# Haochen-Wang409/U2PL

Measured on AMD Instinct MI355X. Metric: train images/sec at 769x769 (R101-DeepLabv3+), higher is better.
Workload: dtype f32

## Files before the change

### u2pl_amd/csrc/common.h

```cpp
#pragma once
#include <hip/hip_runtime.h>
#include <stdint.h>

#define U2PL_API extern "C" __attribute__((visibility("default")))

#define U2PL_LAUNCH_CHECK()                      \
    do {                                         \
        hipError_t e__ = hipGetLastError();      \
        if (e__ != hipSuccess) return (int)e__;  \
    } while (0)

#define U2PL_EINVAL 1001

#include <atomic>
extern std::atomic<unsigned long long> u2pl_kernel_launch_count;
#define U2PL_LAUNCH(...)                        \
    do {                                        \
        u2pl_kernel_launch_count.fetch_add(1, std::memory_order_relaxed);             \
        hipLaunchKernelGGL(__VA_ARGS__);        \
    } while (0)

#ifdef U2PL_HBM_MAXW
#define U2PL_HBM_KERNEL __attribute__((amdgpu_waves_per_eu(1, U2PL_HBM_MAXW)))
#else
#define U2PL_HBM_KERNEL
#endif

static inline int cdiv(long a, long b) { return (int)((a + b - 1) / b); }
static inline int grid_for(long n, int block, int max_blocks = 256 * 16) {
    long g = (n + block - 1) / block;
    if (g > max_blocks) g = max_blocks;
    if (g < 1) g = 1;
    return (int)g;
}

__device__ __forceinline__ float wave_sum(float v) {
#pragma unroll
    for (int o = 32; o > 0; o >>= 1) v += __shfl_xor(v, o, 64);
    return v;
}
template <int CTRL>
__device__ __forceinline__ float dpp_add(float v) {
    return v + __builtin_bit_cast(float, __builtin_amdgcn_update_dpp(0, __builtin_bit_cast(int, v), CTRL, 0xf, 0xf, false));
}
__device__ __forceinline__ float wave_allsum_dpp(float v) {
    v = dpp_add<0x128>(v);
    v = dpp_add<0x124>(v);
    v = dpp_add<0x122>(v);
    v = dpp_add<0x121>(v);
    const int b = __builtin_bit_cast(int, v);
    const float r0 = __builtin_bit_cast(float, __builtin_amdgcn_readlane(b, 0)), r1 = __builtin_bit_cast(float, __builtin_amdgcn_readlane(b, 16));
    const float r2 = __builtin_bit_cast(float, __builtin_amdgcn_readlane(b, 32)), r3 = __builtin_bit_cast(float, __builtin_amdgcn_readlane(b, 48));
    return (r0 + r1) + (r2 + r3);
}
__device__ __forceinline__ float wave_sum_sgpr(float v) {
    v = dpp_add<0x128>(v);
    v = dpp_add<0x124>(v);
    v = dpp_add<0x122>(v);
    v = dpp_add<0x121>(v);
    v += __builtin_bit_cast(float, __builtin_amdgcn_update_dpp(0, __builtin_bit_cast(int, v), 0x142, 0xa, 0xf, false));
    v += __builtin_bit_cast(float, __builtin_amdgcn_update_dpp(0, __builtin_bit_cast(int, v), 0x143, 0xc, 0xf, false));
    return __builtin_bit_cast(float, __builtin_amdgcn_readlane(__builtin_bit_cast(int, v), 63));
}
__device__ __forceinline__ float lane_put(float old, float val, int lane) {
    return (int)(threadIdx.x & 63) == lane ? val : old;
}
__device__ __forceinline__ float lane_get(float v, int lane) {
    return __builtin_bit_cast(float, __builtin_amdgcn_readlane(__builtin_bit_cast(int, v), lane));
}
__device__ __forceinline__ double wave_sum_d(double v) {
#pragma unroll
    for (int o = 32; o > 0; o >>= 1) v += __shfl_xor(v, o, 64);
    return v;
}
__device__ __forceinline__ unsigned wave_sum_u(unsigned v) {
#pragma unroll
    for (int o = 32; o > 0; o >>= 1) v += __shfl_xor(v, o, 64);
    return v;
}
__device__ __forceinline__ float wave_max(float v) {
#pragma unroll
    for (int o = 32; o > 0; o >>= 1) v = fmaxf(v, __shfl_xor(v, o, 64));
    return v;
}

#define U2PL_AMAX_SHARDS 64
#define U2PL_AMAX_STRIDE 32
#define U2PL_AMAX_WORDS (U2PL_AMAX_SHARDS * U2PL_AMAX_STRIDE)
__device__ __forceinline__ unsigned amax_bits(unsigned m, float v) {
    const unsigned b = __float_as_uint(v) & 0x7fffffffu;
    return b > m ? b : m;
}
__device__ __forceinline__ unsigned amax_bits4(unsigned m, float4 v) {
    return amax_bits(amax_bits(amax_bits(amax_bits(m, v.x), v.y), v.z), v.w);
}
__device__ __forceinline__ unsigned wave_max_u(unsigned m) {
#pragma unroll
    for (int o = 32; o > 0; o >>= 1) {
        const unsigned t = (unsigned)__shfl_xor((int)m, o, 64);
        m = t > m ? t : m;
    }
    return m;
}
__device__ __forceinline__ void amax_wave_publish(unsigned m, unsigned* __restrict__ obj) {
    m = wave_max_u(m);
    if ((threadIdx.x & 63) == 0 && m != 0u) {
        const unsigned wave = blockIdx.x * (blockDim.x >> 6) + (threadIdx.x >> 6);
        atomicMax(obj + (wave & (U2PL_AMAX_SHARDS - 1)) * U2PL_AMAX_STRIDE, m);
    }
}
__device__ __forceinline__ unsigned amax_read(const unsigned* __restrict__ obj) {
    const unsigned v = *(const __attribute__((address_space(1))) unsigned*)(obj + (threadIdx.x & 63) * U2PL_AMAX_STRIDE);
    return (unsigned)__builtin_amdgcn_readfirstlane((int)wave_max_u(v));
}

__device__ __forceinline__ void block_count_flush(unsigned cnt, unsigned* __restrict__ dst) {
    __shared__ unsigned s_cnt;
    if (threadIdx.x == 0) s_cnt = 0;
    __syncthreads();
    cnt = wave_sum_u(cnt);
    if ((threadIdx.x & 63) == 0 && cnt) atomicAdd(&s_cnt, cnt);
    __syncthreads();
    if (threadIdx.x == 0 && s_cnt) atomicAdd(dst, s_cnt);
}

__device__ __forceinline__ unsigned f32_key(float f) {
    unsigned u = __float_as_uint(f);
    return (u & 0x80000000u) ? ~u : (u | 0x80000000u);
}
__device__ __forceinline__ float key_f32(unsigned k) {
    unsigned u = (k & 0x80000000u) ? (k & 0x7fffffffu) : ~k;
    return __uint_as_float(u);
}

struct AcCoord {
    int i0, i1;
    float l0, l1;
};
__device__ __forceinline__ AcCoord ac_coord(int dst, float scale, int in_size) {
    AcCoord c;
    float src = __fmul_rn((float)dst, scale);
    c.i0 = (int)src;
    if (c.i0 > in_size - 1) c.i0 = in_size - 1;
    c.i1 = c.i0 + (c.i0 < in_size - 1 ? 1 : 0);
    c.l1 = __fsub_rn(src, (float)c.i0);
    c.l0 = __fsub_rn(1.0f, c.l1);
    return c;
}
static inline float ac_scale_host(long in, long out) {
    return out > 1 ? (float)(in - 1) / (float)(out - 1) : 0.0f;
}
__device__ __forceinline__ int nearest_src(int dst, float scale, int in_size) {
    int s = (int)floorf(__fmul_rn((float)dst, scale));
    return s < in_size - 1 ? s : in_size - 1;
}

typedef unsigned int u32x4 __attribute__((ext_vector_type(4)));
#define OOB_OFF ((int)0x80000000u)
__device__ __forceinline__ __amdgpu_buffer_rsrc_t make_rsrc(const void* p, unsigned bytes) {
    return __builtin_amdgcn_make_buffer_rsrc((void*)p, (short)0, (int)bytes, 0x00020000);
}
__device__ __forceinline__ float4 buf_load4s(__amdgpu_buffer_rsrc_t r, int lane_off, int uniform_off) {
    u32x4 v = __builtin_amdgcn_raw_buffer_load_b128(r, lane_off, uniform_off, 0);
    return make_float4(__uint_as_float(v.x), __uint_as_float(v.y), __uint_as_float(v.z), __uint_as_float(v.w));
}
__device__ __forceinline__ float4 buf_load4(__amdgpu_buffer_rsrc_t r, int byte_off) {
    u32x4 v = __builtin_amdgcn_raw_buffer_load_b128(r, byte_off, 0, 0);
    return make_float4(__uint_as_float(v.x), __uint_as_float(v.y), __uint_as_float(v.z), __uint_as_float(v.w));
}

#define U2PL_GLOBAL __attribute__((address_space(1)))
template <class T>
__device__ __forceinline__ T ldg(const T* p) { return *(const U2PL_GLOBAL T*)p; }

struct BnEpi {
    const float *mean, *invstd, *gamma, *beta, *res;
    long ldr;
    int relu;
    unsigned* y_amax;
};
```

### u2pl_amd/csrc/wino.hip

```cpp
#include "common.h"
#include "u2pl_hip.h"
#include "wino_t.h"

struct WinoGeom {
    int N, H, W, C, dil, Ty, Tx;
    long tiles;
};

__device__ __forceinline__ void tile_coords(const WinoGeom& g, long t, int& n, int& py, int& px, int& ty, int& tx) {
    tx = (int)(t % g.Tx); t /= g.Tx;
    ty = (int)(t % g.Ty); t /= g.Ty;
    px = (int)(t % g.dil); t /= g.dil;
    py = (int)(t % g.dil);
    n = (int)(t / g.dil);
}

template <int MT>
__global__ __launch_bounds__(256) U2PL_HBM_KERNEL void k_wino_input(const float* __restrict__ x, long ldx, unsigned xbytes, WinoGeom g,
                                                    float* __restrict__ V, unsigned* __restrict__ v_amax) {
    constexpr int A = WinoT<MT>::A;
    const int C4 = g.C >> 2;
    long idx = blockIdx.x * (long)blockDim.x + threadIdx.x;
    if (idx >= g.tiles * C4) {
        if (!v_amax) return;
        idx = g.tiles * C4 - 1;
    }
    const int c4 = (int)(idx % C4);
    const long t = idx / C4;
    int n, py, px, ty, tx;
    tile_coords(g, t, n, py, px, ty, tx);
    const __amdgpu_buffer_rsrc_t rx = make_rsrc(x, xbytes);
    const int ldxb = (int)ldx * 4;
    const int iy0 = py + g.dil * (ty * MT - 1), ix0 = px + g.dil * (tx * MT - 1);
    float4 d[A][A];
#pragma unroll
    for (int i = 0; i < A; ++i) {
        const int iy = iy0 + i * g.dil;
        const bool oky = iy >= 0 && iy < g.H;
#pragma unroll
        for (int j = 0; j < A; ++j) {
            const int ix = ix0 + j * g.dil;
            const bool ok = oky && ix >= 0 && ix < g.W;
            const int off = ((n * g.H + iy) * g.W + ix) * ldxb + c4 * 16;
            d[i][j] = buf_load4(rx, ok ? off : OOB_OFF);
        }
    }
#pragma unroll
    for (int j = 0; j < A; ++j) {
        float4 col[A], r[A];
#pragma unroll
        for (int i = 0; i < A; ++i) col[i] = d[i][j];
        WinoT<MT>::bt(col, r);
#pragma unroll
        for (int i = 0; i < A; ++i) d[i][j] = r[i];
    }
    const long comp_stride = g.tiles * (long)g.C;
    float* out = V + t * g.C + c4 * 4;
    unsigned am = 0u;
#pragma unroll
    for (int i = 0; i < A; ++i) {
        float4 r[A];
        WinoT<MT>::bt(d[i], r);
#pragma unroll
        for (int j = 0; j < A; ++j) {
            *(float4*)(out + (long)(i * A + j) * comp_stride) = r[j];
            am = amax_bits4(am, r[j]);
        }
    }
    if (v_amax) amax_wave_publish(am, v_amax);
}

template <int MT>
__device__ __forceinline__ void wino_weight_one(const float* __restrict__ w, int O, int C, int transposed, float* __restrict__ U, long idx) {
    constexpr int A = WinoT<MT>::A;
    const int c = transposed ? (int)(idx / O) : (int)(idx % C), o = transposed ? (int)(idx % O) : (int)(idx / C);
    float gk[3][3];
#pragma unroll
    for (int r = 0; r < 3; ++r)
#pragma unroll
        for (int s = 0; s < 3; ++s) {
            const int rr = transposed ? 2 - r : r, ss = transposed ? 2 - s : s;
            gk[r][s] = w[(((long)o * 3 + rr) * 3 + ss) * C + c];
        }
    float t[A][3];
#pragma unroll
    for (int s = 0; s < 3; ++s) {
        float col[3] = {gk[0][s], gk[1][s], gk[2][s]}, r[A];
        WinoT<MT>::gg(col, r);
#pragma unroll
        for (int i = 0; i < A; ++i) t[i][s] = r[i];
    }
    const long comp_stride = (long)O * C;
    const long base = transposed ? (long)c * O + o : (long)o * C + c;
#pragma unroll
    for (int i = 0; i < A; ++i) {
        float r[A];
        WinoT<MT>::gg(t[i], r);
#pragma unroll
        for (int j = 0; j < A; ++j) U[(long)(i * A + j) * comp_stride + base] = r[j];
    }
}
template <int MT>
__global__ void k_wino_weight(const float* __restrict__ w, int O, int C, int transposed, float* __restrict__ U) {
    const long idx = blockIdx.x * (long)blockDim.x + threadIdx.x;
    if (idx >= (long)O * C) return;
    wino_weight_one<MT>(w, O, C, transposed, U, idx);
}
struct WinoWeightJob { const float* w; float* U; long begin; int O, C, transposed, mt; };
__global__ void k_wino_weight_multi(const WinoWeightJob* __restrict__ jobs, int njobs, long total) {
    for (long i = blockIdx.x * (long)blockDim.x + threadIdx.x; i < total; i += (long)gridDim.x * blockDim.x) {
        int lo = 0, hi = njobs - 1;
        while (lo < hi) {
            const int mid = (lo + hi + 1) >> 1;
            if (jobs[mid].begin <= i) lo = mid; else hi = mid - 1;
        }
        const WinoWeightJob j = jobs[lo];
        if (j.mt == 4) wino_weight_one<4>(j.w, j.O, j.C, j.transposed, j.U, i - j.begin);
        else wino_weight_one<2>(j.w, j.O, j.C, j.transposed, j.U, i - j.begin);
    }
}

template <int MT>
__global__ __launch_bounds__(256) U2PL_HBM_KERNEL void k_wino_output(const float* __restrict__ Mb, WinoGeom g, int O,
                                                     const float* __restrict__ bias, float* __restrict__ y, long ldy,
                                                     float* __restrict__ stats, const float* __restrict__ pivot,
                                                     BnEpi epi) {
    constexpr int A = WinoT<MT>::A;
    __shared__ __attribute__((aligned(16))) float red[2][256][4];
    const int O4 = O >> 2;
    const int tpb = 256 / O4 > 0 ? 256 / O4 : 1;
    long t;
    int o4;
    bool live;
    if (stats) {
        o4 = threadIdx.x % O4;
        const int tl = threadIdx.x / O4;
        t = (long)blockIdx.x * tpb + tl;
        live = tl < tpb && t < g.tiles;
    } else {
        const long idx = blockIdx.x * (long)blockDim.x + threadIdx.x;
        o4 = (int)(idx % O4);
        t = idx / O4;
        live = t < g.tiles;
    }
    float4 s1 = make_float4(0.f, 0.f, 0.f, 0.f), s2 = s1;
    unsigned am = 0u;
    if (live) {
        int n, py, px, ty, tx;
        tile_coords(g, t, n, py, px, ty, tx);
        const long comp_stride = g.tiles * (long)O;
        const float* in = Mb + t * O + o4 * 4;
        float4 m[A][A];
#pragma unroll
        for (int i = 0; i < A; ++i)
#pragma unroll
            for (int j = 0; j < A; ++j) m[i][j] = *(const float4*)(in + (long)(i * A + j) * comp_stride);
        float4 tmp[MT][A];
#pragma unroll
        for (int j = 0; j < A; ++j) {
            float4 col[A], r[MT];
#pragma unroll
            for (int i = 0; i < A; ++i) col[i] = m[i][j];
            WinoT<MT>::at(col, r);
#pragma unroll
            for (int i = 0; i < MT; ++i) tmp[i][j] = r[i];
        }
        const float* bp = bias + o4 * 4;
        const float* pp = pivot + o4 * 4;
        const float4 bv = bias ? make_float4(bp[0], bp[1], bp[2], bp[3]) : make_float4(0.f, 0.f, 0.f, 0.f);
        const float4 pv = (stats && pivot) ? make_float4(pp[0], pp[1], pp[2], pp[3]) : make_float4(0.f, 0.f, 0.f, 0.f);
        const bool bn_on = epi.mean != nullptr;
        float4 mu4 = bv, is4 = bv, ga4 = bv, be4 = bv;
        if (bn_on) {
            mu4 = *(const float4*)(epi.mean + o4 * 4); is4 = *(const float4*)(epi.invstd + o4 * 4);
            ga4 = *(const float4*)(epi.gamma + o4 * 4); be4 = *(const float4*)(epi.beta + o4 * 4);
        }
#pragma unroll
        for (int i = 0; i < MT; ++i) {
            float4 r[MT];
            WinoT<MT>::at(tmp[i], r);
            const int oy = py + g.dil * (ty * MT + i);
#pragma unroll
            for (int j = 0; j < MT; ++j) {
                const int ox = px + g.dil * (tx * MT + j);
                if (oy < g.H && ox < g.W) {
                    float4 v = f4add(r[j], bv);
                    const long pix = (long)(n * g.H + oy) * g.W + ox;
                    if (bn_on) {
                        v.x = (v.x - mu4.x) * is4.x * ga4.x + be4.x; v.y = (v.y - mu4.y) * is4.y * ga4.y + be4.y;
                        v.z = (v.z - mu4.z) * is4.z * ga4.z + be4.z; v.w = (v.w - mu4.w) * is4.w * ga4.w + be4.w;
                        if (epi.res) v = f4add(v, *(const float4*)(epi.res + pix * epi.ldr + o4 * 4));
                        if (epi.relu) { v.x = fmaxf(v.x, 0.f); v.y = fmaxf(v.y, 0.f); v.z = fmaxf(v.z, 0.f); v.w = fmaxf(v.w, 0.f); }
                    }
                    *(float4*)(y + pix * ldy + o4 * 4) = v;
                    am = amax_bits4(am, v);
                    const float4 dv = f4sub(v, pv);
                    s1 = f4add(s1, dv);
                    s2 = f4add(s2, make_float4(dv.x * dv.x, dv.y * dv.y, dv.z * dv.z, dv.w * dv.w));
                }
            }
        }
    }
    if (epi.y_amax) amax_wave_publish(am, epi.y_amax);
    if (!stats) return;
    *(float4*)red[0][threadIdx.x] = s1;
    *(float4*)red[1][threadIdx.x] = s2;
    __syncthreads();
    for (int c = threadIdx.x; c < O; c += 256) {
        float a1 = 0.f, a2 = 0.f;
        for (int tl = 0; tl < tpb; ++tl) {
            a1 += red[0][tl * O4 + (c >> 2)][c & 3];
            a2 += red[1][tl * O4 + (c >> 2)][c & 3];
        }
        stats[(long)blockIdx.x * 2 * O + c] = a1;
        stats[(long)blockIdx.x * 2 * O + O + c] = a2;
    }
}

template <int MT>
__global__ __launch_bounds__(256) U2PL_HBM_KERNEL void k_wino_gy(const float* __restrict__ gy, long ldg, unsigned gbytes, WinoGeom g,
                                                 float* __restrict__ Mg, unsigned* __restrict__ mg_amax) {
    constexpr int A = WinoT<MT>::A;
    const int C4 = g.C >> 2;
    long idx = blockIdx.x * (long)blockDim.x + threadIdx.x;
    if (idx >= g.tiles * C4) {
        if (!mg_amax) return;
        idx = g.tiles * C4 - 1;
    }
    const int c4 = (int)(idx % C4);
    const long t = idx / C4;
    int n, py, px, ty, tx;
    tile_coords(g, t, n, py, px, ty, tx);
    const __amdgpu_buffer_rsrc_t rg = make_rsrc(gy, gbytes);
    const int ldb = (int)ldg * 4;
    float4 v[MT][MT];
#pragma unroll
    for (int i = 0; i < MT; ++i) {
        const int oy = py + g.dil * (ty * MT + i);
#pragma unroll
        for (int j = 0; j < MT; ++j) {
            const int ox = px + g.dil * (tx * MT + j);
            const bool ok = oy < g.H && ox < g.W;
            const int off = ((n * g.H + oy) * g.W + ox) * ldb + c4 * 16;
            v[i][j] = buf_load4(rg, ok ? off : OOB_OFF);
        }
    }
    float4 tmp[A][MT];
#pragma unroll
    for (int j = 0; j < MT; ++j) {
        float4 col[MT], r[A];
#pragma unroll
        for (int i = 0; i < MT; ++i) col[i] = v[i][j];
        WinoT<MT>::av(col, r);
#pragma unroll
        for (int i = 0; i < A; ++i) tmp[i][j] = r[i];
    }
    const long comp_stride = g.tiles * (long)g.C;
    float* out = Mg + t * g.C + c4 * 4;
    unsigned am = 0u;
#pragma unroll
    for (int i = 0; i < A; ++i) {
        float4 r[A];
        WinoT<MT>::av(tmp[i], r);
#pragma unroll
        for (int j = 0; j < A; ++j) {
            *(float4*)(out + (long)(i * A + j) * comp_stride) = r[j];
            am = amax_bits4(am, r[j]);
        }
    }
    if (mg_amax) amax_wave_publish(am, mg_amax);
}

template <int MT>
__global__ __launch_bounds__(256) void k_wino_wgrad_finish(const float* __restrict__ part, int nsplit, int O, int C,
                                                           int accumulate, float* __restrict__ dw) {
    constexpr int A = WinoT<MT>::A;
    const int C4 = C >> 2;
    const long idx = blockIdx.x * (long)blockDim.x + threadIdx.x;
    if (idx >= (long)O * C4) return;
    const int c4 = (int)(idx % C4), o = (int)(idx / C4);
    const long slab = (long)O * A * A * C;
    const float* p = part + (long)o * A * A * C + c4 * 4;
    float4 u[A][A];
#pragma unroll
    for (int i = 0; i < A; ++i)
#pragma unroll
        for (int j = 0; j < A; ++j) u[i][j] = make_float4(0.f, 0.f, 0.f, 0.f);
    for (int z = 0; z < nsplit; ++z) {
        float4 v[A][A];
#pragma unroll
        for (int i = 0; i < A; ++i)
#pragma unroll
            for (int j = 0; j < A; ++j) v[i][j] = *(const float4*)(p + (long)z * slab + (long)(i * A + j) * C);
#pragma unroll
        for (int i = 0; i < A; ++i)
#pragma unroll
            for (int j = 0; j < A; ++j) u[i][j] = f4add(u[i][j], v[i][j]);
    }
    float4 t[3][A];
#pragma unroll
    for (int j = 0; j < A; ++j) {
        float cx[A], cy[A], cz[A], cw[A], rx[3], ry[3], rz[3], rw[3];
#pragma unroll
        for (int i = 0; i < A; ++i) { cx[i] = u[i][j].x; cy[i] = u[i][j].y; cz[i] = u[i][j].z; cw[i] = u[i][j].w; }
        WinoT<MT>::gt(cx, rx); WinoT<MT>::gt(cy, ry); WinoT<MT>::gt(cz, rz); WinoT<MT>::gt(cw, rw);
#pragma unroll
        for (int i = 0; i < 3; ++i) t[i][j] = make_float4(rx[i], ry[i], rz[i], rw[i]);
    }
    const bool vec_ok = (reinterpret_cast<uintptr_t>(dw) & 15) == 0;
#pragma unroll
    for (int r3 = 0; r3 < 3; ++r3) {
        float cx[A], cy[A], cz[A], cw[A], rx[3], ry[3], rz[3], rw[3];
#pragma unroll
        for (int j = 0; j < A; ++j) { cx[j] = t[r3][j].x; cy[j] = t[r3][j].y; cz[j] = t[r3][j].z; cw[j] = t[r3][j].w; }
        WinoT<MT>::gt(cx, rx); WinoT<MT>::gt(cy, ry); WinoT<MT>::gt(cz, rz); WinoT<MT>::gt(cw, rw);
#pragma unroll
        for (int s3 = 0; s3 < 3; ++s3) {
            float* d = dw + (((long)o * 3 + r3) * 3 + s3) * C + c4 * 4;
            float4 val = make_float4(rx[s3], ry[s3], rz[s3], rw[s3]);
            if (vec_ok) {
                if (accumulate) val = f4add(*(const float4*)d, val);
                *(float4*)d = val;
            } else {
                d[0] = accumulate ? d[0] + val.x : val.x; d[1] = accumulate ? d[1] + val.y : val.y;
                d[2] = accumulate ? d[2] + val.z : val.z; d[3] = accumulate ? d[3] + val.w : val.w;
            }
        }
    }
}

static int wino_geom(int N, int H, int W, int C, int dil, int mt, WinoGeom& g) {
    if (mt != 2 && mt != 4) return U2PL_EINVAL;
    if (dil < 1 || C % 4) return U2PL_EINVAL;
    g.N = N; g.H = H; g.W = W; g.C = C; g.dil = dil;
    g.Ty = cdiv(cdiv(H, dil), mt);
    g.Tx = cdiv(cdiv(W, dil), mt);
    g.tiles = (long)N * dil * dil * g.Ty * g.Tx;
    return 0;
}

U2PL_API size_t u2pl_wino_tiles(int N, int H, int W, int dil, int mt) {
    WinoGeom g;
    if (wino_geom(N, H, W, 4, dil, mt, g)) return 0;
    return (size_t)g.tiles;
}
U2PL_API int u2pl_wino_stat_blocks(long tiles, int O) {
    const int tpb = 256 / (O / 4) > 0 ? 256 / (O / 4) : 1;
    return (int)((tiles + tpb - 1) / tpb);
}

static int run_wino_input(const float* x, long ldx, int N, int H, int W, int C, int dil, int mt, float* V, float* v_amax,
                          hipStream_t stream) {
    WinoGeom g;
    if (wino_geom(N, H, W, C, dil, mt, g)) return U2PL_EINVAL;
    const long xb = (((long)N * H * W - 1) * ldx + C) * 4;
    if (xb >= (1L << 31)) return U2PL_EINVAL;
    const long total = g.tiles * (C / 4);
    const dim3 grid((unsigned)cdiv(total, 256)), block(256);
    if (mt == 4) U2PL_LAUNCH(k_wino_input<4>, grid, block, 0, stream, x, ldx, (unsigned)xb, g, V, (unsigned*)v_amax);
    else U2PL_LAUNCH(k_wino_input<2>, grid, block, 0, stream, x, ldx, (unsigned)xb, g, V, (unsigned*)v_amax);
    U2PL_LAUNCH_CHECK();
    return 0;
}
U2PL_API int u2pl_wino_input_f32(const float* x, long ldx, int N, int H, int W, int C, int dil, int mt, float* V,
                                 hipStream_t stream) {
    return run_wino_input(x, ldx, N, H, W, C, dil, mt, V, nullptr, stream);
}
U2PL_API int u2pl_wino_input_amax_f32(const float* x, long ldx, int N, int H, int W, int C, int dil, int mt, float* V, float* v_amax,
                                      hipStream_t stream) {
    return run_wino_input(x, ldx, N, H, W, C, dil, mt, V, v_amax, stream);
}

U2PL_API int u2pl_wino_weight_multi_f32(const void* jobs, int njobs, long total, hipStream_t stream) {
    if (njobs <= 0 || total <= 0) return njobs == 0 ? 0 : U2PL_EINVAL;
    U2PL_LAUNCH(k_wino_weight_multi, dim3(grid_for(total, 256, 4096)), dim3(256), 0, stream, (const WinoWeightJob*)jobs, njobs, total);
    U2PL_LAUNCH_CHECK();
    return 0;
}
U2PL_API int u2pl_wino_weight_f32(const float* w, int O, int C, int transposed, int mt, float* U, hipStream_t stream) {
    if (mt != 2 && mt != 4) return U2PL_EINVAL;
    const dim3 grid((unsigned)cdiv((long)O * C, 256)), block(256);
    if (mt == 4) U2PL_LAUNCH(k_wino_weight<4>, grid, block, 0, stream, w, O, C, transposed, U);
    else U2PL_LAUNCH(k_wino_weight<2>, grid, block, 0, stream, w, O, C, transposed, U);
    U2PL_LAUNCH_CHECK();
    return 0;
}

static int run_wino_output(const float* Mb, int N, int H, int W, int O, int dil, int mt, const float* bias, float* y,
                           long ldy, float* stats_partial, const float* pivot, const BnEpi& epi, hipStream_t stream) {
    WinoGeom g;
    if (wino_geom(N, H, W, O, dil, mt, g)) return U2PL_EINVAL;
    if (stats_partial && (O / 4 > 256 || (O & 3))) return U2PL_EINVAL;
    const long total = g.tiles * (O / 4);
    const unsigned nblk = stats_partial ? (unsigned)u2pl_wino_stat_blocks(g.tiles, O) : (unsigned)cdiv(total, 256);
    if (mt == 4) U2PL_LAUNCH(k_wino_output<4>, dim3(nblk), dim3(256), 0, stream, Mb, g, O, bias, y, ldy, stats_partial, pivot, epi);
    else U2PL_LAUNCH(k_wino_output<2>, dim3(nblk), dim3(256), 0, stream, Mb, g, O, bias, y, ldy, stats_partial, pivot, epi);
    U2PL_LAUNCH_CHECK();
    return 0;
}
U2PL_API int u2pl_wino_output_f32(const float* Mb, int N, int H, int W, int O, int dil, int mt, const float* bias,
                                  float* y, long ldy, float* stats_partial, const float* pivot, hipStream_t stream) {
    const BnEpi off = {nullptr, nullptr, nullptr, nullptr, nullptr, 0, 0, nullptr};
    return run_wino_output(Mb, N, H, W, O, dil, mt, bias, y, ldy, stats_partial, pivot, off, stream);
}
U2PL_API int u2pl_wino_output_bnact_f32(const float* Mb, int N, int H, int W, int O, int dil, int mt, const float* bias,
                                        float* y, long ldy, const float* mean, const float* invstd, const float* gamma,
                                        const float* beta, const float* res, long ldr, int relu, hipStream_t stream) {
    if (!mean || !invstd || !gamma || !beta || (O & 3) || (ldy & 3) || (res && (ldr & 3))) return U2PL_EINVAL;
    const BnEpi epi = {mean, invstd, gamma, beta, res, ldr, relu, nullptr};
    return run_wino_output(Mb, N, H, W, O, dil, mt, bias, y, ldy, nullptr, nullptr, epi, stream);
}
U2PL_API int u2pl_wino_output_bnact_amax_f32(const float* Mb, int N, int H, int W, int O, int dil, int mt, const float* bias,
                                             float* y, long ldy, const float* mean, const float* invstd, const float* gamma,
                                             const float* beta, const float* res, long ldr, int relu, float* y_amax,
                                             hipStream_t stream) {
    if (!mean || !invstd || !gamma || !beta || (O & 3) || (ldy & 3) || (res && (ldr & 3))) return U2PL_EINVAL;
    const BnEpi epi = {mean, invstd, gamma, beta, res, ldr, relu, (unsigned*)y_amax};
    return run_wino_output(Mb, N, H, W, O, dil, mt, bias, y, ldy, nullptr, nullptr, epi, stream);
}

static int run_wino_gy(const float* gy, long ldg, int N, int H, int W, int O, int dil, int mt, float* Mg, float* mg_amax,
                       hipStream_t stream) {
    WinoGeom g;
    if (wino_geom(N, H, W, O, dil, mt, g)) return U2PL_EINVAL;
    const long gb = (((long)N * H * W - 1) * ldg + O) * 4;
    if (gb >= (1L << 31)) return U2PL_EINVAL;
    const long total = g.tiles * (O / 4);
    const dim3 grid((unsigned)cdiv(total, 256)), block(256);
    if (mt == 4) U2PL_LAUNCH(k_wino_gy<4>, grid, block, 0, stream, gy, ldg, (unsigned)gb, g, Mg, (unsigned*)mg_amax);
    else U2PL_LAUNCH(k_wino_gy<2>, grid, block, 0, stream, gy, ldg, (unsigned)gb, g, Mg, (unsigned*)mg_amax);
    U2PL_LAUNCH_CHECK();
    return 0;
}
U2PL_API int u2pl_wino_gy_f32(const float* gy, long ldg, int N, int H, int W, int O, int dil, int mt, float* Mg,
                              hipStream_t stream) {
    return run_wino_gy(gy, ldg, N, H, W, O, dil, mt, Mg, nullptr, stream);
}
U2PL_API int u2pl_wino_gy_amax_f32(const float* gy, long ldg, int N, int H, int W, int O, int dil, int mt, float* Mg, float* mg_amax,
                                   hipStream_t stream) {
    return run_wino_gy(gy, ldg, N, H, W, O, dil, mt, Mg, mg_amax, stream);
}

U2PL_API int u2pl_wino_wgrad_finish_f32(const float* part, int nsplit, int O, int C, int mt, int accumulate, float* dw,
                                        hipStream_t stream) {
    if (mt != 2 && mt != 4) return U2PL_EINVAL;
    if (C % 4) return U2PL_EINVAL;
    const dim3 grid((unsigned)cdiv((long)O * (C / 4), 256)), block(256);
    if (mt == 4) U2PL_LAUNCH(k_wino_wgrad_finish<4>, grid, block, 0, stream, part, nsplit, O, C, accumulate, dw);
    else U2PL_LAUNCH(k_wino_wgrad_finish<2>, grid, block, 0, stream, part, nsplit, O, C, accumulate, dw);
    U2PL_LAUNCH_CHECK();
    return 0;
}
```

Before: 38.29.

## Specialize Winograd input/output kernels with compile-time variants, 32-bit indexing, buffer ops

Templates the Winograd input and output transform kernels on wave-uniform tile ownership, amax and epilogue form, so unused branches (stats, BN, residual, amax) compile away. Index math moves from 64-bit to 32-bit, and the tile index is made scalar via readfirstlane when every wave owns a single tile, which enables scalar-offset buffer loads. Output stores use buffer stores with OOB masking instead of branches, and launch bounds set occupancy targets. In exchange there are more kernel instantiations and new size guards that reject tensors whose offsets exceed 32 bits.

Result: no change. 38.05 (-0.6%).

```diff
diff --git a/u2pl_amd/csrc/common.h b/u2pl_amd/csrc/common.h
--- a/u2pl_amd/csrc/common.h
+++ b/u2pl_amd/csrc/common.h
@@ -169,6 +169,12 @@
     return make_float4(__uint_as_float(v.x), __uint_as_float(v.y), __uint_as_float(v.z), __uint_as_float(v.w));
 }
 
+__device__ __forceinline__ void buf_store4(__amdgpu_buffer_rsrc_t r, int byte_off, float4 v) {
+    u32x4 w;
+    w.x = __float_as_uint(v.x); w.y = __float_as_uint(v.y); w.z = __float_as_uint(v.z); w.w = __float_as_uint(v.w);
+    __builtin_amdgcn_raw_buffer_store_b128(w, r, byte_off, 0, 0);
+}
+
 #define U2PL_GLOBAL __attribute__((address_space(1)))
 template <class T>
 __device__ __forceinline__ T ldg(const T* p) { return *(const U2PL_GLOBAL T*)p; }
diff --git a/u2pl_amd/csrc/wino.hip b/u2pl_amd/csrc/wino.hip
--- a/u2pl_amd/csrc/wino.hip
+++ b/u2pl_amd/csrc/wino.hip
@@ -1,12 +1,29 @@
 #include "common.h"
 #include "u2pl_hip.h"
 #include "wino_t.h"
+#include <type_traits>
 
 struct WinoGeom {
     int N, H, W, C, dil, Ty, Tx;
     long tiles;
 };
 
+#ifdef U2PL_HBM_MAXW
+#define U2PL_WINO_KERNEL(W) __launch_bounds__(256) U2PL_HBM_KERNEL
+#else
+#define U2PL_WINO_KERNEL(W) __launch_bounds__(256, W)
+#endif
+
+__device__ __forceinline__ void tile_coords(const WinoGeom& g, unsigned t, int& n, int& py, int& px, int& ty, int& tx) {
+    const unsigned r = t / (unsigned)g.Tx, q = r / (unsigned)g.Ty;
+    tx = (int)(t - r * (unsigned)g.Tx);
+    ty = (int)(r - q * (unsigned)g.Ty);
+    if (g.dil == 1) { px = 0; py = 0; n = (int)q; return; }
+    const unsigned u = q / (unsigned)g.dil;
+    px = (int)(q - u * (unsigned)g.dil);
+    n = (int)(u / (unsigned)g.dil);
+    py = (int)(u - (unsigned)n * (unsigned)g.dil);
+}
 __device__ __forceinline__ void tile_coords(const WinoGeom& g, long t, int& n, int& py, int& px, int& ty, int& tx) {
     tx = (int)(t % g.Tx); t /= g.Tx;
     ty = (int)(t % g.Ty); t /= g.Ty;
@@ -14,19 +31,36 @@
     py = (int)(t % g.dil);
     n = (int)(t / g.dil);
 }
-
-template <int MT>
-__global__ __launch_bounds__(256) U2PL_HBM_KERNEL void k_wino_input(const float* __restrict__ x, long ldx, unsigned xbytes, WinoGeom g,
+template <bool UNI>
+__device__ __forceinline__ unsigned wave_tile(unsigned t) {
+    return UNI ? (unsigned)__builtin_amdgcn_readfirstlane((int)t) : t;
+}
+typedef float f32x4g __attribute__((ext_vector_type(4)));
+__device__ __forceinline__ float4 plane_load4(const float* base, unsigned long plane, int k, unsigned off) {
+    const f32x4g v = *(const U2PL_GLOBAL f32x4g*)((const U2PL_GLOBAL char*)base + (unsigned long)k * plane + off);
+    return make_float4(v.x, v.y, v.z, v.w);
+}
+__device__ __forceinline__ float4 f4sel(bool c, float4 a, float4 b) {
+    return make_float4(c ? a.x : b.x, c ? a.y : b.y, c ? a.z : b.z, c ? a.w : b.w);
+}
+__device__ __forceinline__ float4 ldg4f(const float* p) { return plane_load4(p, 0, 0, 0u); }
+__device__ __forceinline__ void plane_store4(float* base, unsigned long plane, int k, unsigned off, float4 v) {
+    f32x4g w; w.x = v.x; w.y = v.y; w.z = v.z; w.w = v.w;
+    *(U2PL_GLOBAL f32x4g*)((U2PL_GLOBAL char*)base + (unsigned long)k * plane + off) = w;
+}
+
+template <int MT, bool UNI, bool AMAX>
+__global__ U2PL_WINO_KERNEL(MT == 4 ? 2 : 6) void k_wino_input(const float* __restrict__ x, long ldx, unsigned xbytes, WinoGeom g,
                                                     float* __restrict__ V, unsigned* __restrict__ v_amax) {
     constexpr int A = WinoT<MT>::A;
-    const int C4 = g.C >> 2;
-    long idx = blockIdx.x * (long)blockDim.x + threadIdx.x;
-    if (idx >= g.tiles * C4) {
-        if (!v_amax) return;
-        idx = g.tiles * C4 - 1;
-    }
-    const int c4 = (int)(idx % C4);
-    const long t = idx / C4;
+    const unsigned C4 = (unsigned)g.C >> 2, total = (unsigned)g.tiles * C4;
+    unsigned idx = blockIdx.x * 256u + threadIdx.x;
+    if (idx >= total) {
+        if (!AMAX) return;
+        idx = total - 1;
+    }
+    const unsigned tq = idx / C4, c4 = idx - tq * C4;
+    const unsigned t = wave_tile<UNI>(tq);
     int n, py, px, ty, tx;
     tile_coords(g, t, n, py, px, ty, tx);
     const __amdgpu_buffer_rsrc_t rx = make_rsrc(x, xbytes);
@@ -41,8 +75,9 @@
         for (int j = 0; j < A; ++j) {
             const int ix = ix0 + j * g.dil;
             const bool ok = oky && ix >= 0 && ix < g.W;
-            const int off = ((n * g.H + iy) * g.W + ix) * ldxb + c4 * 16;
-            d[i][j] = buf_load4(rx, ok ? off : OOB_OFF);
+            const int pix = ok ? ((n * g.H + iy) * g.W + ix) * ldxb : 0;
+            if (UNI) d[i][j] = buf_load4s(rx, ok ? (int)(c4 * 16) : OOB_OFF, pix);
+            else d[i][j] = buf_load4(rx, ok ? pix + (int)(c4 * 16) : OOB_OFF);
         }
     }
 #pragma unroll
@@ -54,8 +89,8 @@
 #pragma unroll
         for (int i = 0; i < A; ++i) d[i][j] = r[i];
     }
-    const long comp_stride = g.tiles * (long)g.C;
-    float* out = V + t * g.C + c4 * 4;
+    const unsigned long plane = (unsigned long)g.tiles * g.C * 4;
+    const unsigned off = (t * (unsigned)g.C + c4 * 4) * 4;
     unsigned am = 0u;
 #pragma unroll
     for (int i = 0; i < A; ++i) {
@@ -63,11 +98,11 @@
         WinoT<MT>::bt(d[i], r);
 #pragma unroll
         for (int j = 0; j < A; ++j) {
-            *(float4*)(out + (long)(i * A + j) * comp_stride) = r[j];
-            am = amax_bits4(am, r[j]);
-        }
-    }
-    if (v_amax) amax_wave_publish(am, v_amax);
+            plane_store4(V, plane, i * A + j, off, r[j]);
+            if (AMAX) am = amax_bits4(am, r[j]);
+        }
+    }
+    if (AMAX) amax_wave_publish(am, v_amax);
 }
 
 template <int MT>
@@ -120,41 +155,43 @@
     }
 }
 
-template <int MT>
-__global__ __launch_bounds__(256) U2PL_HBM_KERNEL void k_wino_output(const float* __restrict__ Mb, WinoGeom g, int O,
+enum { WOUT_PLAIN = 0, WOUT_STATS = 1, WOUT_BN = 2, WOUT_BN_AMAX = 3 };
+template <int MT, bool UNI, int FORM>
+__global__ U2PL_WINO_KERNEL(MT == 4 ? 2 : 4) void k_wino_output(const float* __restrict__ Mb, WinoGeom g, int O,
                                                      const float* __restrict__ bias, float* __restrict__ y, long ldy,
-                                                     float* __restrict__ stats, const float* __restrict__ pivot,
-                                                     BnEpi epi) {
+                                                     unsigned ybytes, unsigned rbytes, float* __restrict__ stats,
+                                                     const float* __restrict__ pivot, BnEpi epi) {
     constexpr int A = WinoT<MT>::A;
-    __shared__ __attribute__((aligned(16))) float red[2][256][4];
-    const int O4 = O >> 2;
+    constexpr bool STATS = FORM == WOUT_STATS, BN = FORM == WOUT_BN || FORM == WOUT_BN_AMAX, AMAX = FORM == WOUT_BN_AMAX;
+    __shared__ __attribute__((aligned(16))) float red[STATS ? 2 : 1][STATS ? 256 : 1][4];
+    const unsigned O4 = (unsigned)O >> 2;
     const int tpb = 256 / O4 > 0 ? 256 / O4 : 1;
-    long t;
-    int o4;
+    unsigned tq, o4;
     bool live;
-    if (stats) {
-        o4 = threadIdx.x % O4;
-        const int tl = threadIdx.x / O4;
-        t = (long)blockIdx.x * tpb + tl;
-        live = tl < tpb && t < g.tiles;
+    if (STATS) {
+        const unsigned tl = threadIdx.x / O4;
+        o4 = threadIdx.x - tl * O4;
+        tq = blockIdx.x * (unsigned)tpb + tl;
+        live = tl < (unsigned)tpb && tq < (unsigned)g.tiles;
     } else {
-        const long idx = blockIdx.x * (long)blockDim.x + threadIdx.x;
-        o4 = (int)(idx % O4);
-        t = idx / O4;
-        live = t < g.tiles;
-    }
+        const unsigned idx = blockIdx.x * 256u + threadIdx.x;
+        tq = idx / O4;
+        o4 = idx - tq * O4;
+        live = tq < (unsigned)g.tiles;
+    }
+    const unsigned t = wave_tile<UNI>(tq);
     float4 s1 = make_float4(0.f, 0.f, 0.f, 0.f), s2 = s1;
     unsigned am = 0u;
     if (live) {
         int n, py, px, ty, tx;
         tile_coords(g, t, n, py, px, ty, tx);
-        const long comp_stride = g.tiles * (long)O;
-        const float* in = Mb + t * O + o4 * 4;
+        const unsigned long plane = (unsigned long)g.tiles * O * 4;
+        const unsigned off = (t * (unsigned)O + o4 * 4) * 4;
         float4 m[A][A];
 #pragma unroll
         for (int i = 0; i < A; ++i)
 #pragma unroll
-            for (int j = 0; j < A; ++j) m[i][j] = *(const float4*)(in + (long)(i * A + j) * comp_stride);
+            for (int j = 0; j < A; ++j) m[i][j] = plane_load4(Mb, plane, i * A + j, off);
         float4 tmp[MT][A];
 #pragma unroll
         for (int j = 0; j < A; ++j) {
@@ -168,41 +205,51 @@
         const float* bp = bias + o4 * 4;
         const float* pp = pivot + o4 * 4;
         const float4 bv = bias ? make_float4(bp[0], bp[1], bp[2], bp[3]) : make_float4(0.f, 0.f, 0.f, 0.f);
-        const float4 pv = (stats && pivot) ? make_float4(pp[0], pp[1], pp[2], pp[3]) : make_float4(0.f, 0.f, 0.f, 0.f);
-        const bool bn_on = epi.mean != nullptr;
+        const float4 pv = (STATS && pivot) ? make_float4(pp[0], pp[1], pp[2], pp[3]) : make_float4(0.f, 0.f, 0.f, 0.f);
         float4 mu4 = bv, is4 = bv, ga4 = bv, be4 = bv;
-        if (bn_on) {
-            mu4 = *(const float4*)(epi.mean + o4 * 4); is4 = *(const float4*)(epi.invstd + o4 * 4);
-            ga4 = *(const float4*)(epi.gamma + o4 * 4); be4 = *(const float4*)(epi.beta + o4 * 4);
-        }
-#pragma unroll
-        for (int i = 0; i < MT; ++i) {
-            float4 r[MT];
-            WinoT<MT>::at(tmp[i], r);
-            const int oy = py + g.dil * (ty * MT + i);
-#pragma unroll
-            for (int j = 0; j < MT; ++j) {
-                const int ox = px + g.dil * (tx * MT + j);
-                if (oy < g.H && ox < g.W) {
+        if (BN) {
+            mu4 = ldg4f(epi.mean + o4 * 4); is4 = ldg4f(epi.invstd + o4 * 4);
+            ga4 = ldg4f(epi.gamma + o4 * 4); be4 = ldg4f(epi.beta + o4 * 4);
+        }
+        const __amdgpu_buffer_rsrc_t ry = make_rsrc(y, ybytes);
+        const bool has_res = BN && epi.res != nullptr;
+        const __amdgpu_buffer_rsrc_t rr = make_rsrc(has_res ? (const void*)epi.res : (const void*)y, has_res ? rbytes : 0u);
+        const int ldyb = (int)ldy * 4, ldrb = (int)epi.ldr * 4;
+        auto rows = [&](auto RES) {
+#pragma unroll
+            for (int i = 0; i < MT; ++i) {
+                float4 r[MT];
+                WinoT<MT>::at(tmp[i], r);
+                const int oy = py + g.dil * (ty * MT + i);
+#pragma unroll
+                for (int j = 0; j < MT; ++j) {
+                    const int ox = px + g.dil * (tx * MT + j);
+                    const bool ok = oy < g.H && ox < g.W;
+                    const int pix = ok ? (n * g.H + oy) * g.W + ox : 0;
+                    const int lane = ok ? (int)(o4 * 16) : OOB_OFF;
                     float4 v = f4add(r[j], bv);
-                    const long pix = (long)(n * g.H + oy) * g.W + ox;
-                    if (bn_on) {
+                    if (BN) {
                         v.x = (v.x - mu4.x) * is4.x * ga4.x + be4.x; v.y = (v.y - mu4.y) * is4.y * ga4.y + be4.y;
                         v.z = (v.z - mu4.z) * is4.z * ga4.z + be4.z; v.w = (v.w - mu4.w) * is4.w * ga4.w + be4.w;
-                        if (epi.res) v = f4add(v, *(const float4*)(epi.res + pix * epi.ldr + o4 * 4));
+                        if (decltype(RES)::value)
+                            v = f4add(v, UNI ? buf_load4s(rr, lane, pix * ldrb) : buf_load4(rr, ok ? pix * ldrb + lane : OOB_OFF));
                         if (epi.relu) { v.x = fmaxf(v.x, 0.f); v.y = fmaxf(v.y, 0.f); v.z = fmaxf(v.z, 0.f); v.w = fmaxf(v.w, 0.f); }
                     }
-                    *(float4*)(y + pix * ldy + o4 * 4) = v;
-                    am = amax_bits4(am, v);
-                    const float4 dv = f4sub(v, pv);
-                    s1 = f4add(s1, dv);
-                    s2 = f4add(s2, make_float4(dv.x * dv.x, dv.y * dv.y, dv.z * dv.z, dv.w * dv.w));
+                    buf_store4(ry, ok ? pix * ldyb + lane : OOB_OFF, v);
+                    if (AMAX) am = ok ? amax_bits4(am, v) : am;
+                    if (STATS) {
+                        const float4 dv = f4sub(v, pv);
+                        s1 = f4sel(ok, f4add(s1, dv), s1);
+                        s2 = f4sel(ok, f4add(s2, make_float4(dv.x * dv.x, dv.y * dv.y, dv.z * dv.z, dv.w * dv.w)), s2);
+                    }
                 }
             }
-        }
-    }
-    if (epi.y_amax) amax_wave_publish(am, epi.y_amax);
-    if (!stats) return;
+        };
+        if (has_res) rows(std::integral_constant<bool, true>{});
+        else rows(std::integral_constant<bool, false>{});
+    }
+    if (AMAX) amax_wave_publish(am, epi.y_amax);
+    if (!STATS) return;
     *(float4*)red[0][threadIdx.x] = s1;
     *(float4*)red[1][threadIdx.x] = s2;
     __syncthreads();
@@ -349,16 +396,31 @@
     return (int)((tiles + tpb - 1) / tpb);
 }
 
+static bool wino_fits32(const WinoGeom& g, int C) { return g.tiles * (long)C * 4 < (1L << 32); }
+static bool wave_owns_tile(int C) { return (C / 4) % 64 == 0; }
+template <class F>
+static void wino_dispatch(int mt, bool uni, bool third, F&& f) {
+    auto with_mt = [&](auto MT) {
+        using B0 = std::integral_constant<bool, false>;
+        using B1 = std::integral_constant<bool, true>;
+        if (uni) { if (third) f(MT, B1{}, B1{}); else f(MT, B1{}, B0{}); }
+        else { if (third) f(MT, B0{}, B1{}); else f(MT, B0{}, B0{}); }
+    };
+    if (mt == 4) with_mt(std::integral_constant<int, 4>{});
+    else with_mt(std::integral_constant<int, 2>{});
+}
+
 static int run_wino_input(const float* x, long ldx, int N, int H, int W, int C, int dil, int mt, float* V, float* v_amax,
                           hipStream_t stream) {
     WinoGeom g;
     if (wino_geom(N, H, W, C, dil, mt, g)) return U2PL_EINVAL;
     const long xb = (((long)N * H * W - 1) * ldx + C) * 4;
-    if (xb >= (1L << 31)) return U2PL_EINVAL;
+    if (xb >= (1L << 31) || !wino_fits32(g, C)) return U2PL_EINVAL;
     const long total = g.tiles * (C / 4);
     const dim3 grid((unsigned)cdiv(total, 256)), block(256);
-    if (mt == 4) U2PL_LAUNCH(k_wino_input<4>, grid, block, 0, stream, x, ldx, (unsigned)xb, g, V, (unsigned*)v_amax);
-    else U2PL_LAUNCH(k_wino_input<2>, grid, block, 0, stream, x, ldx, (unsigned)xb, g, V, (unsigned*)v_amax);
+    wino_dispatch(mt, wave_owns_tile(C), v_amax != nullptr, [&](auto MT, auto UNI, auto AMAX) {
+        U2PL_LAUNCH((k_wino_input<decltype(MT)::value, decltype(UNI)::value, decltype(AMAX)::value>), grid, block, 0, stream, x, ldx, (unsigned)xb, g, V, (unsigned*)v_amax);
+    });
     U2PL_LAUNCH_CHECK();
     return 0;
 }
@@ -391,10 +453,20 @@
     WinoGeom g;
     if (wino_geom(N, H, W, O, dil, mt, g)) return U2PL_EINVAL;
     if (stats_partial && (O / 4 > 256 || (O & 3))) return U2PL_EINVAL;
+    const long yb = (((long)N * H * W - 1) * ldy + O) * 4, rb = epi.res ? (((long)N * H * W - 1) * epi.ldr + O) * 4 : 0;
+    if (yb >= (1L << 31) || rb >= (1L << 31) || !wino_fits32(g, O)) return U2PL_EINVAL;
     const long total = g.tiles * (O / 4);
     const unsigned nblk = stats_partial ? (unsigned)u2pl_wino_stat_blocks(g.tiles, O) : (unsigned)cdiv(total, 256);
-    if (mt == 4) U2PL_LAUNCH(k_wino_output<4>, dim3(nblk), dim3(256), 0, stream, Mb, g, O, bias, y, ldy, stats_partial, pivot, epi);
-    else U2PL_LAUNCH(k_wino_output<2>, dim3(nblk), dim3(256), 0, stream, Mb, g, O, bias, y, ldy, stats_partial, pivot, epi);
+    const bool bn = epi.mean != nullptr;
+    wino_dispatch(mt, wave_owns_tile(O), bn ? epi.y_amax != nullptr : stats_partial != nullptr, [&](auto MT, auto UNI, auto T) {
+        const dim3 grid(nblk), block(256);
+        if (bn)
+            U2PL_LAUNCH((k_wino_output<decltype(MT)::value, decltype(UNI)::value, decltype(T)::value ? WOUT_BN_AMAX : WOUT_BN>), grid, block, 0, stream, Mb, g, O, bias, y, ldy,
+                        (unsigned)yb, (unsigned)rb, stats_partial, pivot, epi);
+        else
+            U2PL_LAUNCH((k_wino_output<decltype(MT)::value, decltype(UNI)::value, decltype(T)::value ? WOUT_STATS : WOUT_PLAIN>), grid, block, 0, stream, Mb, g, O, bias, y, ldy,
+                        (unsigned)yb, (unsigned)rb, stats_partial, pivot, epi);
+    });
     U2PL_LAUNCH_CHECK();
     return 0;
 }
```
